# Opendigitalradio/ODR-AudioEnc

Measured on AMD Instinct MI355X. Metric: real-time stereo DAB MP2 streams sustained (frames/s) @128 kbps/48 kHz, higher is better.
Workload: dtype f64; 1 GPU; 4096 streams/GPU x 48 kHz stereo (mode 's') x 128 kbps, psy 1, full encode (BASELINE configs[1]), 32 frames/stream/step; streams_per_gpu=4096, parallelism=streams sharded over 1 GPU(s), no data-path collective

## Files before the change

odr-audioenc_amd/csrc/mp2_alloc.h:

```cpp
#ifndef MP2_WAVE_PARTS
#error "include mp2_wave.h"
#endif
TL_FN int tl_allocate(const TlBlockShared *TL_RESTRICT B, int adb, int nch, int sblimit, int jsbound, PARG(int, a_ln), PARG(int, a_nbal),
                      PARG(int, a_sfs), PARG(int, a_sfs_o), PARG(double, a_smr), PARG(int, ba))
{
    PV(uint64_t, ukey); PV(uint64_t, ukey2); PV(int, nbits); PV(int, cost); PV(int, cost2);
    PV(int, jpair);
    TL_LANES_BEGIN
    const int c = lane & 1, sb = lane >> 1;
    const bool live = c < nch && sb < sblimit;
    const int maxa = (1 << L(a_nbal)) - 1;
    L(ukey) = live ? tl_mnr_key(B->snr_line[L(a_ln)][0] - L(a_smr)) : ~0ull;
    L(ukey2) = (live && 1 < maxa) ? tl_mnr_key(B->snr_line[L(a_ln)][1] - L(a_smr)) : ~0ull;
    L(ba) = 0;
    L(nbits) = (sb < sblimit && c < (sb < jsbound ? nch : 1)) ? L(a_nbal) : 0;
    L(cost) = live ? B->bits12_line[L(a_ln)][1] + 2 + L(a_sfs) + ((nch == 2 && sb >= jsbound) ? 2 + L(a_sfs_o) : 0) : 0;
    L(cost2) = live ? B->bits12_line[L(a_ln)][2] - B->bits12_line[L(a_ln)][1] : 0;
    L(jpair) = (live && nch == 2 && sb >= jsbound) ? 1 : 0;
    TL_LANES_END
    const int bbal = TL_WAVE_SUM_I32(nbits);
    const int ad = adb - (bbal + 16 + 32);
    int spent = 0;
    const bool any_pair = nch == 2 && jsbound < sblimit;
    for (; TL_ENC_LEVEL < 4;) {
        PV(uint64_t, keff); PV(uint64_t, k2eff);
        TL_LANES_BEGIN L(keff) = L(ukey); L(k2eff) = L(ukey2); TL_LANES_END
        if (any_pair) {
            PV(uint64_t, ok1); PV(uint64_t, ok2);
            TL_SWAP1_U64(ok1, ukey); TL_SWAP1_U64(ok2, ukey2);
            TL_LANES_BEGIN
            if (L(jpair)) { if (L(ok1) < L(keff)) L(keff) = L(ok1); if (L(ok2) < L(k2eff)) L(k2eff) = L(ok2); }
            TL_LANES_END
        }
        const uint64_t M = TL_WAVE_MIN_U64(k2eff);
        PV(bool, inb); PV(int, bcost);
        TL_LANES_BEGIN
        L(inb) = L(keff) < M;
        L(bcost) = (L(inb) && !(L(jpair) && (lane & 1))) ? L(cost) : 0;
        TL_LANES_END
        const uint64_t bm = TL_BALLOT(inb);
        if (bm == 0ull) break;
        const int csum = TL_WAVE_SUM_I32(bcost);
        bool last_round = false;
        if (csum > ad - spent) {
            PV(int, pre); PV(int, kh); PV(int, kl); PV(uint64_t, kb);
            TL_LANES_BEGIN L(pre) = 0; L(kh) = (int)(uint32_t)(L(keff) >> 32); L(kl) = (int)(uint32_t)L(keff); L(kb) = L(keff) + 1; TL_LANES_END
            uint64_t pm = bm;
            while (pm) {
                const int j = __builtin_ctzll(pm);
                pm &= pm - 1;
                const int cj = TL_READLANE_I32(bcost, j);
                if (cj == 0) continue;
                const uint64_t kj = ((uint64_t)(uint32_t)TL_READLANE_I32(kh, j) << 32) | (uint32_t)TL_READLANE_I32(kl, j);
                TL_LANES_BEGIN
                if (kj < L(kb)) L(pre) += cj;
                TL_LANES_END
            }
            TL_LANES_BEGIN
            L(inb) = L(inb) && L(pre) <= ad - spent;
            L(bcost) = L(inb) ? L(bcost) : 0;
            TL_LANES_END
            if (TL_BALLOT(inb) == 0ull) break;
            spent += TL_WAVE_SUM_I32(bcost);
            last_round = true;
        } else spent += csum;
        TL_LANES_BEGIN
        if (L(inb)) {
            const int nba = L(ba) + 1;
            L(ba) = nba;
            L(ukey) = L(ukey2);
            L(cost) = L(cost2);
            L(ukey2) = (nba + 1 >= (1 << L(a_nbal)) - 1) ? ~0ull : tl_mnr_key(B->snr_line[L(a_ln)][(nba + 1) & 15] - L(a_smr));
            L(cost2) = B->bits12_line[L(a_ln)][(nba + 2) & 15] - B->bits12_line[L(a_ln)][(nba + 1) & 15];
        }
        TL_LANES_END
        if (last_round) break;
    }
    for (; TL_ENC_LEVEL < 4;) {
        PV(uint64_t, key);
        TL_LANES_BEGIN
        L(key) = L(cost) <= ad - spent ? L(ukey) : ~0ull;
        TL_LANES_END
        const int wl = TL_WAVE_ARGMIN_U64(key);
        if (wl < 0) break;
        const int min_sb = wl >> 1;
        spent += TL_READLANE_I32(cost, wl);
        const bool joint_pair = (min_sb >= jsbound && nch == 2);
        TL_LANES_BEGIN
        if (lane == wl || (joint_pair && (lane ^ 1) == wl)) {
            const int nba = L(ba) + 1;
            L(ba) = nba;
            L(ukey) = L(ukey2);
            L(cost) = L(cost2);
            L(ukey2) = (nba + 1 >= (1 << L(a_nbal)) - 1) ? ~0ull : tl_mnr_key(B->snr_line[L(a_ln)][(nba + 1) & 15] - L(a_smr));
            L(cost2) = B->bits12_line[L(a_ln)][(nba + 2) & 15] - B->bits12_line[L(a_ln)][(nba + 1) & 15];
        }
        TL_LANES_END
    }
    return ad - spent;
}

TL_FN void tl_allocate_pair(const TlBlockShared *TL_RESTRICT B, int adb0, int adb1, int sblimit, PARG(int, a_ln), PARG(int, a_nbal),
                            PARG(int, a_sfs), PARG(double, a_smr), PARG(int, ba))
{
    PV(uint64_t, ukey); PV(uint64_t, ukey2); PV(int, nbits); PV(int, cost); PV(int, cost2); PV(int, room); PV(int, ph); PV(int, bbal);
    TL_LANES_BEGIN
    const bool live = (lane >> 1) < sblimit;
    const int maxa = (1 << L(a_nbal)) - 1;
    L(ukey) = live ? tl_mnr_key(B->snr_line[L(a_ln)][0] - L(a_smr)) : ~0ull;
    L(ukey2) = (live && 1 < maxa) ? tl_mnr_key(B->snr_line[L(a_ln)][1] - L(a_smr)) : ~0ull;
    L(ba) = 0;
    L(nbits) = live ? L(a_nbal) : 0;
    L(cost) = live ? B->bits12_line[L(a_ln)][1] + 2 + L(a_sfs) : 0;
    L(cost2) = live ? B->bits12_line[L(a_ln)][2] - B->bits12_line[L(a_ln)][1] : 0;
    TL_LANES_END
    TL_PAR_SUM_I32(bbal, nbits);
    TL_LANES_BEGIN
    L(room) = ((lane & 1) ? adb1 : adb0) - (L(bbal) + 16 + 32);
    L(ph) = 0;
    TL_LANES_END
    for (; TL_ENC_LEVEL < 4;) {
        PV(uint64_t, k2); PV(uint64_t, M); PV(bool, inb); PV(int, bcost); PV(int, csum); PV(bool, part);
        TL_LANES_BEGIN L(k2) = L(ph) == 0 ? L(ukey2) : ~0ull; TL_LANES_END
        TL_PAR_MIN_U64(M, k2);
        TL_LANES_BEGIN
        L(inb) = L(ph) == 0 && L(ukey) < L(M);
        L(bcost) = L(inb) ? L(cost) | 0x10000 : 0;
        TL_LANES_END
        if (TL_BALLOT(inb) == 0ull) break;
        TL_PAR_SUM_I32(csum, bcost);
        TL_LANES_BEGIN L(part) = L(ph) == 0 && (L(csum) & 0xffff) > L(room); TL_LANES_END
        if (TL_BALLOT(part) != 0ull) {
            PV(int, pre); PV(int, kh); PV(int, kl); PV(bool, pin);
            TL_LANES_BEGIN
            L(pre) = 0; L(kh) = (int)(uint32_t)(L(ukey) >> 32); L(kl) = (int)(uint32_t)L(ukey); L(pin) = L(inb) && L(part);
            TL_LANES_END
            PV(uint64_t, kb);
            for (int u = 0; u < 2; u++) {
                TL_LANES_BEGIN L(kb) = (lane & 1) == u ? L(ukey) + 1 : 0ull; TL_LANES_END
                uint64_t pm = TL_BALLOT(pin) & (0x5555555555555555ull << u);
                while (pm) {
                    const int j = __builtin_ctzll(pm);
                    pm &= pm - 1;
                    const int cj = TL_READLANE_I32(bcost, j) & 0xffff;
                    const uint64_t kj = ((uint64_t)(uint32_t)TL_READLANE_I32(kh, j) << 32) | (uint32_t)TL_READLANE_I32(kl, j);
                    TL_LANES_BEGIN
                    if (kj < L(kb)) L(pre) += cj;
                    TL_LANES_END
                }
            }
            TL_LANES_BEGIN
            if (L(part)) { L(inb) = L(inb) && L(pre) <= L(room); L(bcost) = L(inb) ? L(bcost) : 0; }
            TL_LANES_END
            TL_PAR_SUM_I32(csum, bcost);
        }
        TL_LANES_BEGIN
        if (L(ph) == 0) {
            L(room) -= L(csum) & 0xffff;
            if ((L(csum) >> 16) == 0 || L(part)) L(ph) = 1;
        }
        if (L(inb)) {
            const int nba = L(ba) + 1;
            L(ba) = nba;
            L(ukey) = L(ukey2);
            L(cost) = L(cost2);
            L(ukey2) = (nba + 1 >= (1 << L(a_nbal)) - 1) ? ~0ull : tl_mnr_key(B->snr_line[L(a_ln)][(nba + 1) & 15] - L(a_smr));
            L(cost2) = B->bits12_line[L(a_ln)][(nba + 2) & 15] - B->bits12_line[L(a_ln)][(nba + 1) & 15];
        }
        TL_LANES_END
    }
    for (; TL_ENC_LEVEL < 4;) {
        PV(uint64_t, key); PV(uint64_t, mk); PV(bool, win);
        TL_LANES_BEGIN L(key) = L(cost) <= L(room) ? L(ukey) : ~0ull; TL_LANES_END
        TL_PAR_MIN_U64(mk, key);
        TL_LANES_BEGIN L(win) = L(key) == L(mk) && L(key) != ~0ull; TL_LANES_END
        const uint64_t m = TL_BALLOT(win);
        if (m == 0ull) break;
        const uint64_t m0 = m & 0x5555555555555555ull, m1 = m & 0xaaaaaaaaaaaaaaaaull;
        const int wl0 = m0 ? __builtin_ctzll(m0) : -1, wl1 = m1 ? __builtin_ctzll(m1) : -1;
        const int c0 = wl0 >= 0 ? TL_READLANE_I32(cost, wl0) : 0, c1 = wl1 >= 0 ? TL_READLANE_I32(cost, wl1) : 0;
        TL_LANES_BEGIN
        L(room) -= (lane & 1) ? c1 : c0;
        if (lane == wl0 || lane == wl1) {
            const int nba = L(ba) + 1;
            L(ba) = nba;
            L(ukey) = L(ukey2);
            L(cost) = L(cost2);
            L(ukey2) = (nba + 1 >= (1 << L(a_nbal)) - 1) ? ~0ull : tl_mnr_key(B->snr_line[L(a_ln)][(nba + 1) & 15] - L(a_smr));
            L(cost2) = B->bits12_line[L(a_ln)][(nba + 2) & 15] - B->bits12_line[L(a_ln)][(nba + 1) & 15];
        }
        TL_LANES_END
    }
}
```

odr-audioenc_amd/csrc/mp2_wave.h:

```cpp
#pragma once
#include "mp2_types.h"
#include "tl_libm.h"
#include <math.h>
#include <stddef.h>

#ifdef TL_EMULATE
#define TL_FN static inline
#define TL_LANES_BEGIN for (int lane = 0; lane < 64; ++lane) {
#define TL_LANES_END }
#define TL_SYNC() ((void)0)
#define PV(T, name) T name[64]
#define PA(T, name, n) T name[64][n]
#define L(name) name[lane]
#define PARG(T, name) T (&name)[64]
#define PARGA(T, name, n) T (&name)[64][n]
#define TL_OTHER(name, idx, src) name[src] idx
#define TL_ATOMIC_OR(p, v) (*(p) |= (v))
TL_FN uint64_t tlh_ballot(const bool (&p)[64]) { uint64_t m = 0; for (int i = 0; i < 64; i++) if (p[i]) m |= 1ull << i; return m; }
TL_FN uint64_t tlh_min_u64(const uint64_t (&v)[64]) { uint64_t m = v[0]; for (int i = 1; i < 64; i++) if (v[i] < m) m = v[i]; return m; }
TL_FN int tlh_sum_i32(const int (&v)[64]) { int s = 0; for (int i = 0; i < 64; i++) s += v[i]; return s; }
TL_FN uint32_t tlh_xor_u32(const uint32_t (&v)[64]) { uint32_t s = 0; for (int i = 0; i < 64; i++) s ^= v[i]; return s; }
TL_FN void tlh_exscan_i32(int (&d)[64], const int (&v)[64]) { int s = 0; for (int i = 0; i < 64; i++) { d[i] = s; s += v[i]; } }
TL_FN int tlh_argmin_u64(const uint64_t (&v)[64])
{
    const uint64_t m = tlh_min_u64(v);
    if (m == ~0ull) return -1;
    for (int i = 0; i < 64; i += 2) if (v[i] == m) return i;
    for (int i = 1; i < 64; i += 2) if (v[i] == m) return i;
    return -1;
}
TL_FN void tlh_row16_max_f64(double (&d)[64], const double (&v)[64])
{ for (int r = 0; r < 4; r++) { double m = v[16 * r]; for (int i = 1; i < 16; i++) if (m < v[16 * r + i]) m = v[16 * r + i]; for (int i = 0; i < 16; i++) d[16 * r + i] = m; } }
#define TL_ROW16_MAX_F64(dst, src) tlh_row16_max_f64(dst, src)
TL_FN void tlh_incl_xscan_u32(uint32_t (&d)[64], const uint32_t (&v)[64]) { uint32_t x = 0; for (int i = 0; i < 64; i++) { x ^= v[i]; d[i] = x; } }
#define TL_WAVE_INCL_XSCAN_U32(dst, src) tlh_incl_xscan_u32(dst, src)
TL_FN void tlh_par_min_u64(uint64_t (&d)[64], const uint64_t (&v)[64])
{ for (int p = 0; p < 2; p++) { uint64_t m = v[p]; for (int i = p; i < 64; i += 2) if (v[i] < m) m = v[i]; for (int i = p; i < 64; i += 2) d[i] = m; } }
TL_FN void tlh_par_sum_i32(int (&d)[64], const int (&v)[64])
{ for (int p = 0; p < 2; p++) { int m = 0; for (int i = p; i < 64; i += 2) m += v[i]; for (int i = p; i < 64; i += 2) d[i] = m; } }
#define TL_PAR_MIN_U64(dst, src) tlh_par_min_u64(dst, src)
#define TL_PAR_SUM_I32(dst, src) tlh_par_sum_i32(dst, src)
#define TL_BALLOT(name) tlh_ballot(name)
#define TL_SWAP1_U64(dst, src) do { for (int l_ = 0; l_ < 64; l_++) dst[l_] = src[l_ ^ 1]; } while (0)
#define TL_SWAP1_F64(dst, di, src, si) do { for (int l_ = 0; l_ < 64; l_++) dst[l_] di = src[l_ ^ 1] si; } while (0)
#define TL_SPLAT(dst, di, val) do { for (int l_ = 0; l_ < 64; l_++) dst[l_] di = (val); } while (0)
#define TL_ROT32_F64(dst, src) do { for (int l_ = 0; l_ < 64; l_++) dst[l_] = src[(l_ + 32) & 63]; } while (0)
#define TL_MIRROR_SB_F64(dst, src, n) do { for (int l_ = 0; l_ < 64; l_++) for (int k_ = 0; k_ < (n); k_++) dst[l_][k_] = src[2 * (31 - (l_ >> 1)) + (l_ & 1)][k_]; } while (0)
#define TL_WAVE_ARGMIN_U64(name) tlh_argmin_u64(name)
#define TL_WAVE_MIN_U64(name) tlh_min_u64(name)
#define TL_WAVE_SUM_I32(name) tlh_sum_i32(name)
#define TL_WAVE_XOR_U32(name) tlh_xor_u32(name)
#define TL_WAVE_EXSCAN_I32(dst, src) tlh_exscan_i32(dst, src)
#define TL_UNI_I(x) (x)
#define TL_READLANE_I32(name, l) name[l]
#define TL_RESTRICT
#define TL_SELECT(c, a, b) ((c) ? (a) : (b))
#define TL_LAUNDER(p) ((void)0)
#define TL_KARG const TlLaunch *
#define TL_KEEP(x) ((void)0)
#define TL_PIN(x) ((void)0)
#define TL_TIE(p, v) ((void)0)
#define TL_LD2(p, a, b) do { const double *p_ = (p); (a) = p_[0]; (b) = p_[1]; } while (0)
#define TL_ST2(p, a, b) do { double *p_ = (p); p_[0] = (a); p_[1] = (b); } while (0)
#define TL_RANK_BELOW(mask) __builtin_popcountll((mask) & ((1ull << lane) - 1ull))
TL_FN int tl_sign_bit(double x) { return (int)(tl_d2u(x) >> 63); }
#define TL_SCHED_FENCE() ((void)0)
#define TL_SCT(t, row, j) ((t)[(row) + (j)])
#else
#define TL_FN __device__ __forceinline__
#define TL_LANES_BEGIN { int lane_ = (int)(threadIdx.x & 63u); asm volatile("" : "+v"(lane_)); __builtin_assume(lane_ >= 0 && lane_ < 64); const int lane = lane_;
#define TL_LANES_END } TL_SYNC();
#define TL_SYNC() do { __builtin_amdgcn_fence(__ATOMIC_RELEASE, "wavefront"); __builtin_amdgcn_wave_barrier(); \
                       __builtin_amdgcn_fence(__ATOMIC_ACQUIRE, "wavefront"); } while (0)
#define PV(T, name) T name
#define PA(T, name, n) T name[n]
#define L(name) name
#define PARG(T, name) T &name
#define PARGA(T, name, n) T (&name)[n]
#define TL_OTHER(name, idx, src) tld_shfl_f64(name idx, src)
#define TL_ATOMIC_OR(p, v) atomicOr((p), (v))
TL_FN double tld_shfl_f64(double v, int src) { return __shfl(v, src, 64); }
TL_FN double tld_swap1_f64(double v) {
    const uint64_t u = tl_d2u(v);
    const uint32_t lo = (uint32_t)__builtin_amdgcn_update_dpp(0, (int)(uint32_t)u, 0xB1, 0xf, 0xf, true);
    const uint32_t hi = (uint32_t)__builtin_amdgcn_update_dpp(0, (int)(uint32_t)(u >> 32), 0xB1, 0xf, 0xf, true);
    return tl_u2d(((uint64_t)hi << 32) | lo);
}
struct TldMin { template <class T> static TL_FN T f(T a, T b) { return a < b ? a : b; } };
struct TldAdd { template <class T> static TL_FN T f(T a, T b) { return a + b; } };
struct TldXor { template <class T> static TL_FN T f(T a, T b) { return a ^ b; } };
template <class OP, class T> TL_FN T tld_ladder(T v, const T id)
{
    v = OP::f((T)__builtin_amdgcn_update_dpp((int)id, (int)v, 0x111, 0xf, 0xf, false), v);
    v = OP::f((T)__builtin_amdgcn_update_dpp((int)id, (int)v, 0x112, 0xf, 0xf, false), v);
    v = OP::f((T)__builtin_amdgcn_update_dpp((int)id, (int)v, 0x114, 0xf, 0xf, false), v);
    v = OP::f((T)__builtin_amdgcn_update_dpp((int)id, (int)v, 0x118, 0xf, 0xf, false), v);
    v = OP::f((T)__builtin_amdgcn_update_dpp((int)id, (int)v, 0x142, 0xa, 0xf, false), v);
    v = OP::f((T)__builtin_amdgcn_update_dpp((int)id, (int)v, 0x143, 0xc, 0xf, false), v);
    return v;
}
TL_FN uint32_t tld_min_u32(uint32_t v) { return (uint32_t)__builtin_amdgcn_readlane((int)tld_ladder<TldMin>(v, 0xffffffffu), 63); }
TL_FN uint64_t tld_min_u64(uint64_t v) {
    const uint32_t hi = (uint32_t)(v >> 32), lo = (uint32_t)v;
    const uint32_t mhi = tld_min_u32(hi);
    const uint32_t mlo = tld_min_u32(hi == mhi ? lo : 0xffffffffu);
    return ((uint64_t)mhi << 32) | mlo;
}
TL_FN int tld_incl_scan_i32(int v) { return tld_ladder<TldAdd>(v, 0); }
TL_FN uint32_t tld_incl_xscan_u32(uint32_t x) { return tld_ladder<TldXor>(x, 0u); }
#define TL_WAVE_INCL_XSCAN_U32(dst, src) dst = tld_incl_xscan_u32(src)
TL_FN uint32_t tld_xor_u32(uint32_t x) { return (uint32_t)__builtin_amdgcn_readlane((int)tld_incl_xscan_u32(x), 63); }
TL_FN int tld_sum_i32(int v) { return __builtin_amdgcn_readlane(tld_incl_scan_i32(v), 63); }
TL_FN int tld_exscan_i32(int v) { return tld_incl_scan_i32(v) - v; }
TL_FN int tld_argmin_u64(uint64_t v)
{
    const uint32_t hi = (uint32_t)(v >> 32), lo = (uint32_t)v;
    const uint32_t mhi = tld_min_u32(hi);
    uint64_t m = (uint64_t)__ballot(hi == mhi);
    if (__builtin_popcountll(m) > 1) {
        const uint32_t mlo = tld_min_u32(hi == mhi ? lo : 0xffffffffu);
        if ((mhi & mlo) == 0xffffffffu) return -1;
        m = (uint64_t)__ballot(hi == mhi && lo == mlo);
    } else if (mhi == 0xffffffffu && (uint32_t)__builtin_amdgcn_readlane((int)lo, __builtin_ctzll(m)) == 0xffffffffu) return -1;
    const uint64_t even = m & 0x5555555555555555ull;
    return __builtin_ctzll(even ? even : m);
}
template <int SH> TL_FN double tld_row_shr_f64(double v)
{
    const uint64_t u = tl_d2u(v);
    const uint32_t lo = (uint32_t)__builtin_amdgcn_update_dpp((int)(uint32_t)u, (int)(uint32_t)u, 0x110 | SH, 0xf, 0xf, false);
    const uint32_t hi = (uint32_t)__builtin_amdgcn_update_dpp((int)(uint32_t)(u >> 32), (int)(uint32_t)(u >> 32), 0x110 | SH, 0xf, 0xf, false);
    return tl_u2d(((uint64_t)hi << 32) | lo);
}
TL_FN double tld_row16_max_f64(double v)
{
    double o;
    o = tld_row_shr_f64<1>(v); v = v < o ? o : v;
    o = tld_row_shr_f64<2>(v); v = v < o ? o : v;
    o = tld_row_shr_f64<4>(v); v = v < o ? o : v;
    o = tld_row_shr_f64<8>(v); v = v < o ? o : v;
    return v;
}
#define TL_ROW16_MAX_F64(dst, src) dst = tld_row16_max_f64(src)
TL_FN uint32_t tld_par_min_u32(uint32_t v)
{
    uint32_t t;
    t = (uint32_t)__builtin_amdgcn_update_dpp((int)v, (int)v, 0x122, 0xf, 0xf, false); v = t < v ? t : v;
    t = (uint32_t)__builtin_amdgcn_update_dpp((int)v, (int)v, 0x124, 0xf, 0xf, false); v = t < v ? t : v;
    t = (uint32_t)__builtin_amdgcn_update_dpp((int)v, (int)v, 0x128, 0xf, 0xf, false); v = t < v ? t : v;
    const auto r = __builtin_amdgcn_permlane16_swap(v, v, false, false); v = r[0] < r[1] ? r[0] : r[1];
    const auto q = __builtin_amdgcn_permlane32_swap(v, v, false, false); v = q[0] < q[1] ? q[0] : q[1];
    return v;
}
TL_FN uint64_t tld_par_min_u64(uint64_t v)
{
    const uint32_t hi = (uint32_t)(v >> 32), lo = (uint32_t)v;
    const uint32_t mhi = tld_par_min_u32(hi);
    const uint32_t mlo = tld_par_min_u32(hi == mhi ? lo : 0xffffffffu);
    return ((uint64_t)mhi << 32) | mlo;
}
TL_FN int tld_par_sum_i32(int v)
{
    v += __builtin_amdgcn_update_dpp(v, v, 0x122, 0xf, 0xf, false);
    v += __builtin_amdgcn_update_dpp(v, v, 0x124, 0xf, 0xf, false);
    v += __builtin_amdgcn_update_dpp(v, v, 0x128, 0xf, 0xf, false);
    const auto r = __builtin_amdgcn_permlane16_swap((unsigned)v, (unsigned)v, false, false); v = (int)(r[0] + r[1]);
    const auto q = __builtin_amdgcn_permlane32_swap((unsigned)v, (unsigned)v, false, false); v = (int)(q[0] + q[1]);
    return v;
}
#define TL_PAR_MIN_U64(dst, src) dst = tld_par_min_u64(src)
#define TL_PAR_SUM_I32(dst, src) dst = tld_par_sum_i32(src)
#define TL_BALLOT(name) ((uint64_t)__ballot(name))
#define TL_SWAP1_U64(dst, src) dst = tl_d2u(tld_swap1_f64(tl_u2d(src)))
#define TL_SWAP1_F64(dst, di, src, si) dst di = tld_swap1_f64(src si)
#define TL_SPLAT(dst, di, val) dst di = (val)
#define TL_ROT32_F64(dst, src) dst = __shfl(src, (int)((threadIdx.x + 32u) & 63u), 64)
#define TL_MIRROR_SB_F64(dst, src, n) do { const int lane_ = (int)(threadIdx.x & 63u), partner_ = 2 * (31 - (lane_ >> 1)) + (lane_ & 1); \
                                           _Pragma("unroll") for (int k_ = 0; k_ < (n); k_++) dst[k_] = __shfl(src[k_], partner_, 64); } while (0)
#define TL_WAVE_ARGMIN_U64(name) tld_argmin_u64(name)
#define TL_WAVE_MIN_U64(name) tld_min_u64(name)
#define TL_WAVE_SUM_I32(name) tld_sum_i32(name)
#define TL_WAVE_XOR_U32(name) tld_xor_u32(name)
#define TL_WAVE_EXSCAN_I32(dst, src) dst = tld_exscan_i32(src)
#define TL_UNI_I(x) __builtin_amdgcn_readfirstlane(x)
#define TL_READLANE_I32(name, l) __builtin_amdgcn_readlane(name, l)
#define TL_RESTRICT __restrict__
#define TL_SELECT(c, a, b) (__builtin_unpredictable(c) ? (a) : (b))
#define TL_KEEP(x) asm volatile("" : : "v"(x))
typedef double tl_f64x2 __attribute__((ext_vector_type(2)));
#define TL_LD2(p, a, b) do { const tl_f64x2 v_ = *(const tl_f64x2 *)(p); (a) = v_.x; (b) = v_.y; } while (0)
#define TL_ST2(p, a, b) do { tl_f64x2 v_; v_.x = (a); v_.y = (b); *(tl_f64x2 *)(p) = v_; } while (0)
#define TL_RANK_BELOW(mask) ((int)__builtin_amdgcn_mbcnt_hi((uint32_t)((mask) >> 32), __builtin_amdgcn_mbcnt_lo((uint32_t)(mask), 0u)))
#if defined(__HIP_DEVICE_COMPILE__)
typedef const __attribute__((address_space(4))) struct TlLaunch *TlKArg;
#else
typedef const struct TlLaunch *TlKArg;
#endif
#define TL_KARG TlKArg
#define TL_LAUNDER(p) asm volatile("" : "+s"(p))
#define TL_TIE(p, v) asm volatile("" : "+s"(p), "+v"(v))
TL_FN int tl_sign_bit(double x) { int r; asm("v_lshrrev_b32 %0, 31, %1" : "=v"(r) : "v"((uint32_t)(tl_d2u(x) >> 32))); return r; }
#define TL_SCHED_FENCE() __builtin_amdgcn_sched_barrier(0)
#define TL_SCT(t, row, j) ((t)[((row) >> 1) + ((j) & 1) + 220 * ((j) >> 1)])
#define TL_PIN(x) asm volatile("" : "+v"(x))
#endif

#ifndef TL_PRIO_CHAIN
#define TL_PRIO_CHAIN 3
#endif
#ifndef TL_PS_FHT
#define TL_PS_FHT 0
#endif
#ifndef TL_PS_THR
#define TL_PS_THR 1
#endif
#ifndef TL_PS_FB
#define TL_PS_FB 0
#endif
#ifndef TL_PS_Q
#define TL_PS_Q 0
#endif
#ifndef TL_PS_POW
#define TL_PS_POW 1
#endif
#ifndef TL_PRIO_SERIAL
#define TL_PRIO_SERIAL 2
#endif
#ifdef TL_EMULATE
#define TL_PRIO(n) ((void)0)
#define TL_PRIO2(n) ((void)0)
#else
#define TL_PRIO(n) do { if (TL_PRIO_CHAIN) __builtin_amdgcn_s_setprio((n) ? TL_PRIO_CHAIN : TL_PRIO_SERIAL); } while (0)
#define TL_PRIO2(n) do { if (TL_PRIO_SERIAL) __builtin_amdgcn_s_setprio((n) ? TL_PRIO_SERIAL : 0); } while (0)
#endif
#ifdef TL_EMULATE
#define TL_STAMP(sp, k) ((void)0)
#else
#define TL_STAMP(sp, k) do { if (sp) { long long t_ = (long long)__builtin_amdgcn_s_memtime(); if ((threadIdx.x & 63u) == 0) (sp)[k] = t_; } } while (0)
#endif

#if defined(TL_EMULATE) && defined(TL_DEBUG_DUMP)
#include <stdio.h>
#include <stdlib.h>
#define TL_DBG_DUMP(tag, ch, nt, nn, x, b) do { if (getenv("TL_DUMP")) { printf("%s ch%d ntone %d nnoise %d:", tag, ch, nt, nn); \
    for (int i_ = 0; i_ < (nt) + (nn); i_++) printf(" (%.17g,%.6f)", (x)[i_], (b)[i_]); printf("\n"); } } while (0)
#define TL_DBG_WALK(ch, lane, cnt) do { if (getenv("TL_DUMP_WALK")) printf("walk ch%d lane %d cnt %d\n", ch, lane, cnt); } while (0)
static long tl_dbg_rounds = 0, tl_dbg_tones = 0, tl_dbg_deadheads = 0, tl_dbg_fronts = 0, tl_dbg_cands = 0;
#define TL_DBG_CAND(n) (tl_dbg_cands += (n))
#define TL_DBG_ROUND() (tl_dbg_rounds++)
#define TL_DBG_TONES(n, dh) (tl_dbg_tones += (n), tl_dbg_deadheads += (dh) ? 1 : 0, tl_dbg_fronts++)
static long tl_dbg_back[7] = {0, 0, 0, 0, 0, 0, 0};
#define TL_DBG_BACK(k) (tl_dbg_back[k]++)
extern "C" __attribute__((weak, visibility("default"))) void emu_back_stats(long *out) { for (int i = 0; i < 7; i++) out[i] = tl_dbg_back[i]; }
#else
#define TL_DBG_BACK(k) ((void)0)
#define TL_DBG_DUMP(tag, ch, nt, nn, x, b) ((void)0)
#define TL_DBG_WALK(ch, lane, cnt) ((void)0)
#define TL_DBG_ROUND() ((void)0)
#define TL_DBG_TONES(n, dh) ((void)0)
#define TL_DBG_CAND(n) ((void)0)
#endif
#ifndef TL_EXP_LEVEL
#define TL_EXP_LEVEL 0
#endif
#ifndef TL_ENC_LEVEL
#define TL_ENC_LEVEL 0
#endif
#ifndef TL_P2_LEVEL
#define TL_P2_LEVEL 0
#endif
#ifndef TL_P2_SUB
#define TL_P2_SUB 0
#endif
#ifndef TL_P3_NOTAIL
#define TL_P3_NOTAIL 0
#endif
#define TL_DBMIN (-200.0)
#define TL_POWERNORM 90.3090
#define TL_T_NOISE 10
#define TL_T_TONE 20
#define TL_LAST (-1)
#define TL_STOP (-100)

#define TL_CAND_MAX 256
#ifndef TL_FB_BATCH_MAIN
#define TL_FB_BATCH_MAIN 6
#endif
#define TL_PSY_EXT 5
#define TL_TONE_MAX 77
#define TL_MASKER_MAX 128
#define TL_FFT_WORDS (513 + 520)
#define TL_PX(w) ((w).u.fft + 513)
#define TL_EX(i) ((i) ^ (((i) >> 4) & 15))
#define TL_YP_ROW 18
struct TlMainLds {
    static constexpr int kFbBatch = TL_FB_BATCH_MAIN;
    union alignas(16) {
        struct { int16_t pcm[2][TL_HIST + 1152]; } fbk;
        uint32_t frame[2][TL_MAX_FRAME_WORDS + 2];
    } u;
    alignas(16) double yp[TL_FB_BATCH_MAIN][TL_YP_ROW * 3 + 16];
    double smr[2][32];
    double psy_m[2][32];
    int16_t ncentre[32];
    uint8_t scf[2][3][32];
    uint8_t jscale[3][32];
    uint8_t scfsi[2][32];
    uint8_t balloc[2][32];
    uint8_t minidx[2][32];
    uint8_t xpad[TL_MAX_XPAD];
    typedef double (*YpRows)[TL_YP_ROW * 3 + 16];
};
#ifndef TL_Q_REDEAL
#define TL_Q_REDEAL 1
#endif
#ifndef TL_Q_REDEAL_MAX
#define TL_Q_REDEAL_MAX 48
#endif
struct alignas(16) TlQCell { double a, b, s2nf; uint32_t w0, w1; };
struct alignas(16) TlQGran { double s[12]; double sf, rsf; };
#define TL_QRD_OFF ((4 * (TL_MAX_FRAME_WORDS + 2) + 15) & ~15)
#define TL_QRD_CELLS(w) ((TlQCell *)((char *)&(w) + TL_QRD_OFF))
#define TL_QRD_GRANS(w) ((TlQGran *)((char *)&(w) + TL_QRD_OFF + TL_Q_REDEAL_MAX * sizeof(TlQCell)))
static_assert(sizeof(TlQCell) == 32 && sizeof(TlQGran) == 112, "records are whole 16-byte pieces");
static_assert(offsetof(TlMainLds, u) == 0 && offsetof(TlMainLds, yp) == sizeof(((TlMainLds *)0)->u) && offsetof(TlMainLds, yp) % 16 == 0,
              "yp[] follows the staging union without a gap");
static_assert(TL_QRD_OFF + TL_Q_REDEAL_MAX * (sizeof(TlQCell) + sizeof(TlQGran)) <= offsetof(TlMainLds, yp) + sizeof(((TlMainLds *)0)->yp),
              "cell records and granule blocks end inside yp[]");
static_assert(TL_Q_REDEAL_MAX >= 0 && TL_Q_REDEAL_MAX <= 64 && TL_MAX_FRAME_BYTES * 8 / 12 < (1 << 11), "a rank per lane; o_smp fits its 11 bits");
struct alignas(16) TlPsy2Lds {
    struct { double fft[1024]; } u;
    double px[536];
};
struct TlPsyLds {
    struct { double fft[TL_FFT_WORDS]; } u;
    double tone_x[TL_TONE_MAX];
    double nsum[32];
    uint32_t cinfo[TL_CAND_MAX];
    int16_t conf_c[TL_TONE_MAX];
    int16_t conf_nxt[TL_TONE_MAX];
    int16_t tlist[TL_TONE_MAX];
    int16_t ncentre[32];
    int16_t bandoff[40];
    uint8_t ptype[520];
};
#define TL_MK_X(w) ((w).u.fft)
#define TL_MK_BARK(w) ((w).u.fft + TL_MASKER_MAX)
#define TL_LTG(w) ((w).u.fft + 2 * TL_MASKER_MAX)
struct TlMasker { double bark, av, g, c17, n; };
#define TL_MK4(w) ((TlMasker *)((w).u.fft + 2 * TL_MASKER_MAX + 136))
static_assert(2 * TL_MASKER_MAX + 136 + 5 * TL_MASKER_MAX <= TL_FFT_WORDS, "masker records fit the transform buffer");
#define TL_P1B_LIST 32
#define TL_P1B_BASE 700
#define TL_P1B_MKX(w) ((w).u.fft + TL_P1B_BASE)
#define TL_P1B_MKBARK(w) ((w).u.fft + TL_P1B_BASE + 64)
#define TL_P1B_TONE_X(w) ((w).u.fft + TL_P1B_BASE + 128)
#define TL_P1B_PTYPE(w) ((uint8_t *)((w).u.fft + TL_P1B_BASE + 128 + TL_TONE_MAX))
#define TL_P1B_CONF_C(w) ((int16_t *)((w).u.fft + TL_P1B_BASE + 128 + TL_TONE_MAX + 65))
static_assert(TL_P1B_LIST + 27 <= 64 && 2 * TL_MASKER_MAX + 136 + 5 * (TL_P1B_LIST + 27) <= TL_P1B_BASE, "channel 1's masker records end below channel 0's records");
static_assert(TL_P1B_BASE + 128 + TL_TONE_MAX + 65 + (2 * TL_TONE_MAX + 7) / 8 <= TL_FFT_WORDS, "channel 0's records fit the transform buffer");



#ifdef TL_EMULATE
static long tl_emu_near1_full = 0;
#define TL_DBG_NEAR1_FULL() (tl_emu_near1_full++)
#else
#define TL_DBG_NEAR1_FULL() ((void)0)
#endif
#ifdef TL_EMULATE
static long tl_emu_redeal[2][66];
#define TL_DBG_REDEAL(took, ba) do { int n_ = 0; for (int l_ = 0; l_ < 64; l_++) n_ += (ba)[l_] != 0; \
                                     tl_emu_redeal[(took) ? 1 : 0][0]++; tl_emu_redeal[(took) ? 1 : 0][1 + n_]++; } while (0)
extern "C" __attribute__((weak, visibility("default"))) void emu_redeal_stats(long *out)
{ out[0] = tl_emu_redeal[0][0]; out[1] = tl_emu_redeal[1][0]; for (int i = 0; i < 65; i++) { out[2 + i] = tl_emu_redeal[0][1 + i]; out[67 + i] = tl_emu_redeal[1][1 + i]; } }
#else
#define TL_DBG_REDEAL(took, ba) ((void)0)
#endif

#define MP2_WAVE_PARTS 1
#include "mp2_dbsum.h"
#include "mp2_fht.h"
#include "mp2_psy13.h"
#include "mp2_psy24.h"
#include "mp2_fb.h"
#include "mp2_alloc.h"
#include "mp2_pack.h"
#include "mp2_units.h"
#undef MP2_WAVE_PARTS
```

Measured before the change: 36.84 million frames/s.

## Replace serial per-lane prefix-cost scan in bit allocation cut with bisection probes

When a round of greedy bit allocation overflows the budget, the old code walked every candidate lane serially, using a readlane and a wave-wide compare for each one to build prefix costs. The new helper first runs up to a fixed number of pivot probes that split candidates by key, admitting groups whose summed cost fits and discarding keys above the cut. Only the unresolved remainder falls back to the serial prefix scan. This is meant to cut the number of serial wave iterations in the overflow path, at the cost of extra ballots and reductions per probe and a more complicated equivalence argument.

```diff
diff --git a/odr-audioenc_amd/csrc/mp2_alloc.h b/odr-audioenc_amd/csrc/mp2_alloc.h
--- a/odr-audioenc_amd/csrc/mp2_alloc.h
+++ b/odr-audioenc_amd/csrc/mp2_alloc.h
@@ -1,6 +1,67 @@
 #ifndef MP2_WAVE_PARTS
 #error "include mp2_wave.h"
 #endif
+#ifndef TL_ALLOC_CUT_PROBES
+#define TL_ALLOC_CUT_PROBES 12
+#endif
+#ifdef TL_EMULATE
+static long tl_emu_cut[48];
+static int tl_emu_cut_cap = TL_ALLOC_CUT_PROBES;
+#define TL_ALLOC_CUT_CAP tl_emu_cut_cap
+#define TL_DBG_CUT(k, n) (tl_emu_cut[k] += (n))
+#define TL_DBG_CUT_ADMIT(m) (tl_emu_cut[4] += (m) == 0ull)
+extern "C" __attribute__((weak, visibility("default"))) void emu_alloc_cut_stats(long *out) { for (int i = 0; i < 48; i++) out[i] = tl_emu_cut[i]; }
+extern "C" __attribute__((weak, visibility("default"))) void emu_alloc_cut_set_cap(int n) { tl_emu_cut_cap = n < 0 ? TL_ALLOC_CUT_PROBES : n; }
+#else
+#define TL_ALLOC_CUT_CAP TL_ALLOC_CUT_PROBES
+#define TL_DBG_CUT(k, n) ((void)0)
+#define TL_DBG_CUT_ADMIT(m) ((void)0)
+#endif
+TL_FN bool tl_alloc_cut(PARG(uint64_t, keff), PARG(int, bcost), const int room, PARG(int, pre), uint64_t &kout, int &base)
+{
+    PV(int, kh); PV(int, kl); PV(bool, t); PV(int, pc);
+    TL_LANES_BEGIN
+    L(pre) = 0; L(kh) = (int)(uint32_t)(L(keff) >> 32); L(kl) = (int)(uint32_t)L(keff);
+    L(t) = L(bcost) != 0;
+    TL_LANES_END
+    uint64_t um = TL_BALLOT(t);
+    kout = ~0ull; base = 0;
+    int probes = 0;
+    TL_DBG_CUT(0, 1); TL_DBG_CUT(5, __builtin_popcountll(um));
+#pragma nounroll
+    for (; um != 0ull && probes < TL_ALLOC_CUT_CAP; probes++) {
+        const int p = __builtin_ctzll(um);
+        const uint64_t kp = ((uint64_t)(uint32_t)TL_READLANE_I32(kh, p) << 32) | (uint32_t)TL_READLANE_I32(kl, p);
+        TL_LANES_BEGIN L(t) = L(keff) <= kp; TL_LANES_END
+        const uint64_t lm = TL_BALLOT(t) & um;
+        TL_LANES_BEGIN L(pc) = TL_IN_MASK(lm) ? L(bcost) : 0; TL_LANES_END
+        const int s = base + TL_WAVE_SUM_I32(pc);
+        if (s <= room) { base = s; um &= ~lm; }
+        else {
+            kout = kp;
+            TL_LANES_BEGIN L(t) = L(keff) < kp; TL_LANES_END
+            um &= TL_BALLOT(t);
+        }
+    }
+    TL_DBG_CUT(1, probes); TL_DBG_CUT(8 + (probes < 39 ? probes : 39), 1);
+    uint64_t pm = um;
+    if (pm == 0ull) return false;
+    TL_DBG_CUT(2, 1);
+    PV(uint64_t, kb);
+    TL_LANES_BEGIN L(kb) = L(keff) + 1; TL_LANES_END
+    while (pm) {
+        const int j = __builtin_ctzll(pm);
+        pm &= pm - 1;
+        const int cj = TL_READLANE_I32(bcost, j);
+        const uint64_t kj = ((uint64_t)(uint32_t)TL_READLANE_I32(kh, j) << 32) | (uint32_t)TL_READLANE_I32(kl, j);
+        TL_LANES_BEGIN
+        if (kj < L(kb)) L(pre) += cj;
+        TL_LANES_END
+        TL_DBG_CUT(3, 1);
+    }
+    return true;
+}
+
 TL_FN int tl_allocate(const TlBlockShared *TL_RESTRICT B, int adb, int nch, int sblimit, int jsbound, PARG(int, a_ln), PARG(int, a_nbal),
                       PARG(int, a_sfs), PARG(int, a_sfs_o), PARG(double, a_smr), PARG(int, ba))
 {
@@ -43,25 +104,16 @@
         const int csum = TL_WAVE_SUM_I32(bcost);
         bool last_round = false;
         if (csum > ad - spent) {
-            PV(int, pre); PV(int, kh); PV(int, kl); PV(uint64_t, kb);
-            TL_LANES_BEGIN L(pre) = 0; L(kh) = (int)(uint32_t)(L(keff) >> 32); L(kl) = (int)(uint32_t)L(keff); L(kb) = L(keff) + 1; TL_LANES_END
-            uint64_t pm = bm;
-            while (pm) {
-                const int j = __builtin_ctzll(pm);
-                pm &= pm - 1;
-                const int cj = TL_READLANE_I32(bcost, j);
-                if (cj == 0) continue;
-                const uint64_t kj = ((uint64_t)(uint32_t)TL_READLANE_I32(kh, j) << 32) | (uint32_t)TL_READLANE_I32(kl, j);
-                TL_LANES_BEGIN
-                if (kj < L(kb)) L(pre) += cj;
-                TL_LANES_END
-            }
-            TL_LANES_BEGIN
-            L(inb) = L(inb) && L(pre) <= ad - spent;
+            PV(int, pre);
+            uint64_t kout; int base;
+            const bool fell = tl_alloc_cut(keff, bcost, ad - spent, pre, kout, base);
+            TL_LANES_BEGIN
+            L(inb) = L(inb) && L(keff) < kout && base + L(pre) <= ad - spent;
             L(bcost) = L(inb) ? L(bcost) : 0;
             TL_LANES_END
+            TL_DBG_CUT_ADMIT(TL_BALLOT(inb));
             if (TL_BALLOT(inb) == 0ull) break;
-            spent += TL_WAVE_SUM_I32(bcost);
+            spent += fell ? TL_WAVE_SUM_I32(bcost) : base;
             last_round = true;
         } else spent += csum;
         TL_LANES_BEGIN
diff --git a/odr-audioenc_amd/csrc/mp2_wave.h b/odr-audioenc_amd/csrc/mp2_wave.h
--- a/odr-audioenc_amd/csrc/mp2_wave.h
+++ b/odr-audioenc_amd/csrc/mp2_wave.h
@@ -41,6 +41,7 @@
 #define TL_PAR_MIN_U64(dst, src) tlh_par_min_u64(dst, src)
 #define TL_PAR_SUM_I32(dst, src) tlh_par_sum_i32(dst, src)
 #define TL_BALLOT(name) tlh_ballot(name)
+#define TL_IN_MASK(m) ((((m) >> lane) & 1ull) != 0ull)
 #define TL_SWAP1_U64(dst, src) do { for (int l_ = 0; l_ < 64; l_++) dst[l_] = src[l_ ^ 1]; } while (0)
 #define TL_SWAP1_F64(dst, di, src, si) do { for (int l_ = 0; l_ < 64; l_++) dst[l_] di = src[l_ ^ 1] si; } while (0)
 #define TL_SPLAT(dst, di, val) do { for (int l_ = 0; l_ < 64; l_++) dst[l_] di = (val); } while (0)
@@ -171,6 +172,7 @@
 #define TL_PAR_MIN_U64(dst, src) dst = tld_par_min_u64(src)
 #define TL_PAR_SUM_I32(dst, src) dst = tld_par_sum_i32(src)
 #define TL_BALLOT(name) ((uint64_t)__ballot(name))
+#define TL_IN_MASK(m) __builtin_amdgcn_inverse_ballot_w64(m)
 #define TL_SWAP1_U64(dst, src) dst = tl_d2u(tld_swap1_f64(tl_u2d(src)))
 #define TL_SWAP1_F64(dst, di, src, si) dst di = tld_swap1_f64(src si)
 #define TL_SPLAT(dst, di, val) dst di = (val)
```

Measured after the change: 37.20 million frames/s, median of 6. No clear change (+1.0%).
